# Aedelon/MASt3R-SLAM

Hardware: AMD Instinct MI355X
Metric: keyframe-pairs/sec (512x512 two-view infer+match+GN) (higher is better)
Workload: dtype fp16

## Files before the change

### include/m3slam_model.h

```cpp
#ifndef M3SLAM_MODEL_H
#define M3SLAM_MODEL_H

#include <stdint.h>

#ifdef __cplusplus
extern "C" {
#endif

enum { M3_DT_BF16 = 0, M3_DT_F16 = 1, M3_DT_F16_PVBF16 = 2 };

enum {
    M3_EPI_BF16 = 0,
    M3_EPI_BF16_GELU = 1,
    M3_EPI_F32 = 2,
    M3_EPI_F32_ACCUM = 3,
    M3_EPI_BF16_RELU = 4,
    M3_EPI_BF16_ADD = 5,
    M3_EPI_BF16_ROPE = 6,
    M3_EPI_INPUT_RELU = 0x100
};

typedef struct m3_gemm_desc {
    const void *A, *W, *W1;
    const float *bias, *bias1;
    void *C;
    const void *R;
    const int32_t *rope_pos;
    void *c16;
    float *stats_out;
    const float *ln_stats, *ln_colsum, *ln_colsum1;
    const void *r_lo;
    void *c_lo;
    int64_t a_gstride, c_gstride, ln_gstride, stats_gstride;
    int32_t M, N, K, ldc, epilogue, dtype, groups;
    int32_t tokens_per_image, rope_cols, q_cols, ln_slots;
    float rope_base, q_scale, ln_eps;
    int32_t stats_slots;
    int32_t rope_max_pos;
} m3_gemm_desc;
int m3_gemm_ex(const m3_gemm_desc *desc, void *stream);
int m3_gemm_pick_tile(int M, int N, int groups);
int m3_gemm_set_tile(int tile);
int m3_ln_slot_count(int M, int N, int groups);

int m3_conv3x3_grouped2_dt(const void *X, const void *W0, const void *W1, const float *bias0, const float *bias1,
                           void *Y, const void *R, const void *zero16, int B, int H, int Wd, int Cin, int Cout,
                           int stride, int epilogue, void *splitk_ws, int64_t splitk_ws_bytes, int dtype,
                           void *stream);

int64_t m3_conv3x3_splitk_bytes(int B, int H, int Wd, int Cin, int Cout, int stride);

int m3_conv3x3_relu_head4_dt(const void *X, const void *W, const float *bias, const void *W4, const float *b4,
                             float *pts, float *conf, const void *zero16, int B, int H, int Wd, int Cin,
                             int dtype, void *stream);

int m3_dpt_tail_grouped2_dt(const void *X, const void *Wc0, const void *Wc1, const float *bias0, const float *bias1,
                            const void *W40, const void *W41, const float *b40, const float *b41, float *pts,
                            float *conf, const void *zero16, int B, int H, int Wd, int upsample, int dtype,
                            void *stream);

int m3_conv3x3_up_direct_grouped2_dt(const void *X, const void *W0, const void *W1, const float *bias0,
                                     const float *bias1, void *Y, const void *zero16, int B, int H, int Wd, int Cin,
                                     int upsample, int dtype, void *stream);

int m3_conv3x3_direct_grouped2_dt(const void *X, const void *W0, const void *W1, const float *bias0, const float *bias1,
                                  void *Y, const void *R, const void *zero16, int B, int H, int Wd, int Cin, int Cout,
                                  int epilogue, int dtype, void *stream);

int m3_attention_dt(const void *Q, const void *K, const void *V, void *O, int q_row_stride,
                    int kv_row_stride, int o_row_stride, int64_t q_batch_stride,
                    int64_t kv_batch_stride, int64_t o_batch_stride, int nbatch, int heads,
                    int Tq, int Tk, int kv_batch_shift, float scale, int dtype, void *stream);

int m3_attention_prescaled_dt(const void *Q, const void *K, const void *V, void *O, int q_row_stride,
                              int kv_row_stride, int o_row_stride, int64_t q_batch_stride,
                              int64_t kv_batch_stride, int64_t o_batch_stride, int nbatch, int heads,
                              int Tq, int Tk, int kv_batch_shift, int dtype, void *stream);

int m3_rope2d_dt(void *X, const int32_t *pos_yx, const float *cos_sin, int row_stride, int tokens,
                 int heads, int tokens_per_image, int dtype, void *stream);

int m3_layernorm_dt(const float *x, const float *gamma, const float *beta, void *y, int M, int C,
                    float eps, int dtype, void *stream);

int m3_layernorm_grouped2_dt(const float *x, const float *gamma0, const float *beta0, const float *gamma1,
                             const float *beta1, void *y, int M, int C, int in_row_shift, float eps,
                             int dtype, void *stream);
int m3_layernorm_hl_dt(const void *hi, const void *lo, const float *gamma0, const float *beta0, const float *gamma1,
                       const float *beta1, void *y, int rows, int C, int split, float eps, int dtype, void *stream);
int m3_layernorm_dual2_dt(const float *x, const float *ga0, const float *ba0, const float *ga1, const float *ba1,
                          const float *gb0, const float *bb0, const float *gb1, const float *bb1, void *y_own,
                          void *y_cross, int M, int C, float eps, int dtype, void *stream);

int m3_patchify16_dt(const uint8_t *img, void *A, int B, int H, int W, int dtype, void *stream);

int m3_cast_f32_dt(const float *x, void *y, int64_t n, int dtype, void *stream);
int m3_cast16(const void *x, void *y, int64_t n, int from_dtype, int to_dtype, void *stream);
int m3_relu_bf16(const void *x, void *y, int64_t n, void *stream);
int m3_add_dt(const void *a, const void *b, void *y, int64_t n, int dtype, void *stream);
int m3_concat2_bf16(const void *a, const void *b, void *out, int64_t M, int Ca, int Cb, void *stream);
typedef struct m3_pack_seg { const void *src; int64_t dst_off; int64_t nbytes; int32_t mode; int32_t reserved; } m3_pack_seg;
int m3_pack_fields(void *dst, const m3_pack_seg *segs, int nseg, void *stream);
int m3_unshuffle_bf16(const void *in, void *out, int B, int h, int w, int s, int C, int Cpad, void *stream);
int m3_upsample2x_dt(const void *in, void *out, int B, int H, int W, int C, int dtype, void *stream);
int m3_add_upsample2x_dt(const void *low, const void *y, void *out, int B, int H, int W, int OH, int OW, int C,
                         int dtype, void *stream);
int m3_pts_post(const float *in, float *pts, float *conf, int64_t P, void *stream);
int m3_desc_post_dt(const void *in, float *desc, float *dconf, int B, int H, int W, int dtype, void *stream);
int m3_desc_post_f16(const void *in, void *desc_f16, float *dconf, int B, int H, int W, int dtype, void *stream);

#ifdef __cplusplus
}
#endif
#endif
```

### mast3r-slam_amd/csrc/gemm.hip

```cpp
#include <atomic>
#include "gemm_common.h"
#include <cmath>
#include <stdlib.h>

using namespace m3gemm;

namespace {

constexpr int BM = 128, BN = 128;
constexpr int kThreads = 256;

#ifndef M3_GEMM64_STAGES
#define M3_GEMM64_STAGES 2
#endif
constexpr int k_gemm_stages(int T) { return T == 64 ? M3_GEMM64_STAGES : 2; }

template <int MODE , int EPI, int T, int DT, bool SLICED = false>
__global__ void __launch_bounds__(kThreads)
k_gemm(const GemmArgs gin) {
    constexpr int BM = T, BN = T;
    constexpr int NT = T / 32;
    constexpr int kStageBytes = (BM + BN) * BK * 2;
    constexpr int STAGES = k_gemm_stages(T);
    static_assert(4 * (NT == 4 ? 9216 : 4608) + BM * 8 + kRopeTableRows * 128 <= STAGES * kStageBytes, "row table + RoPE table behind the scratch");
    GemmArgs g = select_group<EPI>(gin, blockIdx.y);
    extern __shared__ __attribute__((aligned(16))) unsigned char lds[];
    const int tid = threadIdx.x, lane = tid & 63, wave = tid >> 6;
    const int wr = wave >> 1, wc = wave & 1;
    int kt0 = 0, nk = g.K / BK;
    if (EPI == EPI_F32 && g.splits > 1) {
        const int all = nk, s = blockIdx.z;
        kt0 = (int)((long long)all * s / g.splits);
        nk = (int)((long long)all * (s + 1) / g.splits) - kt0;
        g.C = reinterpret_cast<float *>(g.C) + (size_t)s * g.M * g.ldc;
    }

    const int tiles_n = (g.N + BN - 1) / BN, tiles_m = (g.M + BM - 1) / BM;
    const int nwg = tiles_m * tiles_n;
    const int bid = xcd_remap(blockIdx.x, nwg);
    const int tm = bid / tiles_n, tn = bid % tiles_n;
    const int m0 = tm * BM, n0 = tn * BN;

    const int srow = tid >> 3, sch = (tid & 7) ^ ((srow >> 1) & 7);
    const bf16_t *a_src[NT];
    const bf16_t *w_src[NT];
    int a_oy[NT], a_ox[NT];
    const bf16_t *a_img[NT];
#pragma unroll
    for (int i = 0; i < NT; ++i) {
        int m = m0 + i * 32 + srow;
        m = m < g.M ? m : g.M - 1;
        int n = n0 + i * 32 + srow;
        n = n < g.N ? n : g.N - 1;
        w_src[i] = g.W + (size_t)n * g.K + sch * 8;
        if (MODE == 0) {
            a_src[i] = g.A + (size_t)m * g.K + sch * 8;
        } else {
            const int pix = g.OH * g.OW;
            const int b = m / pix, rem = m - b * pix;
            a_oy[i] = (rem / g.OW) * g.stride - 1;
            a_ox[i] = (rem % g.OW) * g.stride - 1;
            a_img[i] = g.A + (size_t)b * g.H * g.Wd * g.Cin + sch * 8;
        }
    }
    auto stage = [&](int kt, int buf) {
        kt += kt0;
        unsigned char *base = lds + buf * kStageBytes;
        int ky = 0, kx = 0, c0 = 0;
        if (MODE == 1) {
            const int q = kt / 9, tap = kt - q * 9;
            c0 = q * BK;
            ky = tap / 3; kx = tap - ky * 3;
        }
#pragma unroll
        for (int i = 0; i < NT; ++i) {
            const void *src;
            if (MODE == 0) {
                src = a_src[i] + (size_t)kt * BK;
            } else {
                const int iy = a_oy[i] + ky, ix = a_ox[i] + kx;
                const bool in = (iy >= 0) && (iy < g.H) && (ix >= 0) && (ix < g.Wd);
                src = in ? (const void *)(a_img[i] + ((size_t)iy * g.Wd + ix) * g.Cin + c0) : (const void *)g.zero16;
            }
            glds16(src, base + i * 4096 + wave * 1024);
        }
        const size_t koff = MODE == 1 ? conv_k_offset(kt, g.Cin) : (size_t)kt * BK;
#pragma unroll
        for (int i = 0; i < NT; ++i)
            glds16(w_src[i] + koff, base + BM * BK * 2 + i * 4096 + wave * 1024);
    };

    f32x4 acc[NT][NT];
#pragma unroll
    for (int i = 0; i < NT; ++i)
#pragma unroll
        for (int j = 0; j < NT; ++j) acc[i][j] = f32x4{0.f, 0.f, 0.f, 0.f};

    const int frow = lane & 15, fch = lane >> 4;

    constexpr bool CAN_SLICE = SLICED;
    static_assert(!SLICED || (MODE == 1 && T == 128), "sliced accumulation: convolutions on 128 x 128 tiles");
    f32x4 tot[CAN_SLICE ? NT : 1][CAN_SLICE ? NT : 1];
    const int slices = CAN_SLICE ? g.slices : 1;
    int slice = 0, slice_end = slices > 1 ? (int)((long long)nk * 1 / slices) : nk;

    float4 ln_mr = make_float4(0.f, 0.f, 0.f, 0.f);
    if (MODE == 0 && g.ln_stats) {
        const LnLoads L = ln_row_issue<BM>(g, m0, tid);
#pragma unroll
        for (int t0 = 0; t0 < STAGES - 1; ++t0)
            if (t0 < nk) stage(t0, t0);
        ln_mr = ln_row_finish<BM>(g, L, m0, tid);
    } else {
#pragma unroll
        for (int t0 = 0; t0 < STAGES - 1; ++t0)
            if (t0 < nk) stage(t0, t0);
    }
    for (int kt = 0; kt < nk; ++kt) {
        const int buf = kt & (STAGES - 1);
        if (kt + STAGES - 1 < nk) stage(kt + STAGES - 1, (kt + STAGES - 1) & (STAGES - 1));
        const int ahead = nk - 1 - kt < STAGES - 1 ? nk - 1 - kt : STAGES - 1;
        if constexpr (STAGES == 2) {
            if (ahead) {
                if constexpr (NT == 4) asm volatile("s_waitcnt vmcnt(8)" ::: "memory");
                else asm volatile("s_waitcnt vmcnt(4)" ::: "memory");
            } else asm volatile("s_waitcnt vmcnt(0)" ::: "memory");
        } else {
            static_assert(STAGES == 2 || (STAGES == 4 && NT == 2), "vmcnt immediates below are for 4 loads per tile");
            if (ahead == 3) asm volatile("s_waitcnt vmcnt(12)" ::: "memory");
            else if (ahead == 2) asm volatile("s_waitcnt vmcnt(8)" ::: "memory");
            else if (ahead == 1) asm volatile("s_waitcnt vmcnt(4)" ::: "memory");
            else asm volatile("s_waitcnt vmcnt(0)" ::: "memory");
        }
        lds_barrier();
        const unsigned char *As = lds + buf * kStageBytes;
        const unsigned char *Ws = As + BM * BK * 2;
#pragma unroll
        for (int ks = 0; ks < 2; ++ks) {
            bf16x8 af[NT], wf[NT];
#pragma unroll
            for (int i = 0; i < NT; ++i) {
                const int ra = wr * (T / 2) + i * 16 + frow;
                const int ca = (ks * 4 + fch) ^ ((ra >> 1) & 7);
                af[i] = *reinterpret_cast<const bf16x8 *>(As + ra * 128 + ca * 16);
                const int rw = wc * (T / 2) + i * 16 + frow;
                const int cw = (ks * 4 + fch) ^ ((rw >> 1) & 7);
                wf[i] = *reinterpret_cast<const bf16x8 *>(Ws + rw * 128 + cw * 16);
            }
            if (MODE == 1 && g.relu_a) {
#pragma unroll
                for (int i = 0; i < NT; ++i) af[i] = relu_frag(af[i]);
            }
#pragma unroll
            for (int i = 0; i < NT; ++i)
#pragma unroll
                for (int j = 0; j < NT; ++j)
                    acc[i][j] = mfma16<DT>(wf[j], af[i], acc[i][j]);
        }
        lds_barrier();
        if constexpr (CAN_SLICE) {
            if (slices > 1 && kt + 1 == slice_end) {
#pragma unroll
                for (int i = 0; i < NT; ++i)
#pragma unroll
                    for (int j = 0; j < NT; ++j) {
                        tot[i][j] = slice == 0 ? acc[i][j] : tot[i][j] + acc[i][j];
                        acc[i][j] = f32x4{0.f, 0.f, 0.f, 0.f};
                    }
                ++slice;
                slice_end = (int)((long long)nk * (slice + 1) / slices);
            }
        }
    }
    if constexpr (CAN_SLICE) {
        if (slices > 1) {
#pragma unroll
            for (int i = 0; i < NT; ++i)
#pragma unroll
                for (int j = 0; j < NT; ++j) acc[i][j] = tot[i][j];
        }
    }

    if constexpr (EPI == EPI_RELU_HEAD4) {
        static_assert(T == 128, "head fusion needs the 128-wide tile");
        const int r = lane & 15, gq = lane >> 4;
        float part[NT][4];
#pragma unroll
        for (int i = 0; i < NT; ++i)
#pragma unroll
            for (int o = 0; o < 4; ++o) part[i][o] = 0.f;
#pragma unroll
        for (int j = 0; j < NT; ++j) {
            const int n = wc * 64 + j * 16 + gq * 4;
            const float4 b = g.bias ? *reinterpret_cast<const float4 *>(g.bias + n) : make_float4(0.f, 0.f, 0.f, 0.f);
            float w4[4][4];
#pragma unroll
            for (int o = 0; o < 4; ++o) {
                const uint2 q = *reinterpret_cast<const uint2 *>(g.W2 + (size_t)o * g.N + n);
                w4[o][0] = lo16<DT>(q.x); w4[o][1] = hi16<DT>(q.x); w4[o][2] = lo16<DT>(q.y); w4[o][3] = hi16<DT>(q.y);
            }
#pragma unroll
            for (int i = 0; i < NT; ++i) {
                const f32x4 a = acc[i][j];
                const float h[4] = {fmaxf(a[0] + b.x, 0.f), fmaxf(a[1] + b.y, 0.f), fmaxf(a[2] + b.z, 0.f), fmaxf(a[3] + b.w, 0.f)};
#pragma unroll
                for (int o = 0; o < 4; ++o)
                    part[i][o] += (h[0] * w4[o][0] + h[1] * w4[o][1]) + (h[2] * w4[o][2] + h[3] * w4[o][3]);
            }
        }
#pragma unroll
        for (int i = 0; i < NT; ++i)
#pragma unroll
            for (int o = 0; o < 4; ++o) {
                float v = part[i][o];
                v += __shfl_xor(v, 16, 64);
                v += __shfl_xor(v, 32, 64);
                part[i][o] = v;
            }
        float *red = reinterpret_cast<float *>(lds);
        if (wc == 1 && gq == 0) {
#pragma unroll
            for (int i = 0; i < NT; ++i)
                *reinterpret_cast<float4 *>(red + (wr * 64 + i * 16 + r) * 4) =
                    make_float4(part[i][0], part[i][1], part[i][2], part[i][3]);
        }
        __syncthreads();
        if (wc == 0 && gq == 0) {
            float *pts = reinterpret_cast<float *>(g.C);
#pragma unroll
            for (int i = 0; i < NT; ++i) {
                const int m = m0 + wr * 64 + i * 16 + r;
                if (m >= g.M) continue;
                const float4 q = *reinterpret_cast<const float4 *>(red + (wr * 64 + i * 16 + r) * 4);
                const float x = part[i][0] + q.x + g.bias2[0], y = part[i][1] + q.y + g.bias2[1];
                const float z = part[i][2] + q.z + g.bias2[2], c = part[i][3] + q.w + g.bias2[3];
                const float d = sqrtf(x * x + y * y + z * z);
                const float sc = expm1f(d) / fmaxf(d, 1e-8f);
                pts[3 * (size_t)m + 0] = x * sc; pts[3 * (size_t)m + 1] = y * sc; pts[3 * (size_t)m + 2] = z * sc;
                g.C2[m] = 1.0f + expf(c);
            }
        }
    } else {
        float2 *lnt = nullptr;
        if (MODE == 0 && g.ln_stats) {
            lnt = reinterpret_cast<float2 *>(lds + 4 * (NT == 4 ? 9216 : 4608));
            ln_table_store<BM>(lnt, ln_mr, tid);
            __syncthreads();
        }
        const float *ropet = nullptr;
        if constexpr (EPI == EPI_BF16_ROPE && MODE == 0) {
            if (g.rope_pos && g.rope_pmax > 0) {
                float *tab = reinterpret_cast<float *>(lds + 4 * (NT == 4 ? 9216 : 4608) + BM * 8);
                rope_table_build(g, tab, tid, kThreads);
                __syncthreads();
                ropet = tab;
            }
        }
        epilogue_rows<EPI, NT, NT, DT, (EPI == EPI_BF16_ROPE && T == 128) ? 2 : 4>(g, acc, lds + wave * (NT == 4 ? 9216 : 4608), m0 + wr * (T / 2),
                                                                                  n0 + wc * (T / 2), lane, lnt, wr * (T / 2), ropet);
        if constexpr (MODE == 0 && (EPI == EPI_F32 || EPI == EPI_F32_ACCUM)) {
            if (g.stats_out) {
                __syncthreads();
                stats_tile_finalize<BM, NT, NT, 2>(g, lds, NT == 4 ? 9216 : 4608, stats_stage_offset<NT>(), m0, n0, tid);
            }
        }
    }
}

template <int MODE, int T, int DT>
int launch_dt(const GemmArgs &a, int epi, hipStream_t st) {
    constexpr int kLdsBytes = k_gemm_stages(T) * (2 * T) * BK * 2;
    const int tiles = m3_cdiv(a.M, T) * m3_cdiv(a.N, T);
    dim3 grid(tiles, a.groups > 1 ? a.groups : 1, a.splits > 1 ? a.splits : 1), blk(kThreads);
#define M3_L(E) case E: hipLaunchKernelGGL((k_gemm<MODE, E, T, DT>), grid, blk, kLdsBytes, st, a); break
    if (a.slices > 1) {
        if constexpr (MODE == 1 && T == 128) {
            switch (epi) {
                case EPI_BF16: hipLaunchKernelGGL((k_gemm<1, EPI_BF16, 128, DT, true>), grid, blk, kLdsBytes, st, a); break;
                case EPI_BF16_RELU: hipLaunchKernelGGL((k_gemm<1, EPI_BF16_RELU, 128, DT, true>), grid, blk, kLdsBytes, st, a); break;
                case EPI_BF16_ADD: hipLaunchKernelGGL((k_gemm<1, EPI_BF16_ADD, 128, DT, true>), grid, blk, kLdsBytes, st, a); break;
                default: return M3_ERR_INVALID_ARG;
            }
        } else return M3_ERR_INVALID_ARG;
    } else
    if (epi == EPI_RELU_HEAD4) {
        if constexpr (MODE == 1 && T == 128) hipLaunchKernelGGL((k_gemm<1, EPI_RELU_HEAD4, 128, DT>), grid, blk, kLdsBytes, st, a);
        else return M3_ERR_INVALID_ARG;
    } else
    switch (epi) {
        M3_L(EPI_BF16); M3_L(EPI_BF16_GELU); M3_L(EPI_F32); M3_L(EPI_F32_ACCUM); M3_L(EPI_BF16_RELU); M3_L(EPI_BF16_ADD); M3_L(EPI_BF16_ROPE);
        default: return M3_ERR_INVALID_ARG;
    }
#undef M3_L
    M3_CHECK_LAUNCH("m3_gemm");
    return M3_OK;
}

template <int MODE, int T = 128>
int launch(const GemmArgs &a, int epi, hipStream_t st) {
    return a.dt == DT_F16 ? launch_dt<MODE, T, DT_F16>(a, epi, st) : launch_dt<MODE, T, DT_BF16>(a, epi, st);
}

static const double kCost64 = [] { const char *e = getenv("M3_GEMM_COST64"); return e ? atof(e) : 3.2; }();
static std::atomic<int> g_forced_tile{[] { const char *e = getenv("M3_GEMM_TILE"); return e ? atoi(e) : 0; }()};
int pick_tile(int M, int N, int groups = 1, bool dense = true) {
    const int forced = g_forced_tile.load(std::memory_order_relaxed);
    const bool can192 = dense && N % 192 == 0;
    if (forced == 128 || forced == 256) return forced;
    if (forced == 192) return can192 ? 192 : 256;
    const long t256 = (long)m3_cdiv(M, 256) * m3_cdiv(N, 256) * groups, t128 = (long)m3_cdiv(M, 128) * m3_cdiv(N, 128) * groups;
    const double c256 = (double)((t256 + 255) / 256) * 4.0 / 1.4, c128 = (double)((t128 + 511) / 512) * 2.0;
    double c192 = 1e30;
    if (can192) {
        const long t192 = (long)m3_cdiv(M, 256) * (N / 192) * groups;
        c192 = (double)((t192 + 255) / 256) * 3.0 / 1.4 * 1.02;
    }
    double c64 = 1e30;
    if (dense) {
        const long t64 = (long)m3_cdiv(M, 64) * m3_cdiv(N, 64) * groups;
        c64 = (double)((t64 + 1023) / 1024) * 2.0 * 0.25 * kCost64;
    }
    if (forced == 64) return dense ? 64 : 128;
    if (c64 < c128 && c64 < c256 && c64 < c192) return 64;
    if (c192 < c256 && c192 < c128) return 192;
    return c256 < c128 ? 256 : 128;
}
bool use_256(int M, int N, int groups = 1) { return pick_tile(M, N, groups, false) == 256; }

int pick_splits(int pix_per_image, int N, int K) {
    const long tiles = (long)m3_cdiv(pix_per_image, BM) * m3_cdiv(N, BN);
    const int nk = K / BK;
    if (nk < 8) return 1;
    long s = 64 / tiles;
    if (s > nk / 4) s = nk / 4;
    if (s > 16) s = 16;
    return s < 2 ? 1 : (int)s;
}

template <int EPI, int DT>
__global__ void __launch_bounds__(256)
k_splitk_finish(const GemmArgs gin, const float *__restrict__ part, int S) {
    const GemmArgs g = select_group<EPI>(gin, blockIdx.y);
    part += (size_t)blockIdx.y * S * gin.M * gin.N;
    const int nq = g.N / 4;
    const long q = (long)blockIdx.x * 256 + threadIdx.x;
    const int m = (int)(q / nq), n = (int)(q - (long)m * nq) * 4;
    if (m >= g.M) return;
    const size_t plane = (size_t)g.M * g.N;
    const float *p = part + (size_t)m * g.N + n;
    float4 a = *reinterpret_cast<const float4 *>(p);
    for (int s = 1; s < S; ++s) {
        const float4 b = *reinterpret_cast<const float4 *>(p + s * plane);
        a.x += b.x; a.y += b.y; a.z += b.z; a.w += b.w;
    }
    store_tile<EPI, DT>(g, f32x4{a.x, a.y, a.z, a.w}, m, n);
}

template <int MODE>
int run_split(const GemmArgs &a, int S, int epi, void *ws, hipStream_t st) {
    if (MODE == 1 && (epi == EPI_BF16 || epi == EPI_BF16_RELU || epi == EPI_BF16_ADD)) {
        const long tiles = (long)m3_cdiv(a.M, BM) * m3_cdiv(a.N, BN) * (a.groups > 1 ? a.groups : 1);
        static const bool sliced_ok = [] { const char *e = getenv("M3_CONV_SLICED"); return !(e && atoi(e) == 0); }();
        if (sliced_ok && tiles >= m3_device_cu_count()) {
            GemmArgs q = a;
            q.slices = S; q.splits = 1;
            return launch<MODE>(q, epi, st);
        }
    }
    GemmArgs p = a;
    p.C = ws; p.ldc = a.N; p.bias = nullptr; p.bias2 = nullptr; p.R = nullptr; p.splits = S;
    p.c_gstride = (long long)S * a.M * a.N;
    const int rc = launch<MODE>(p, EPI_F32, st);
    if (rc != M3_OK) return rc;
    const dim3 grid((unsigned)m3_cdiv((long)a.M * (a.N / 4), 256L), a.groups > 1 ? a.groups : 1);
#define M3_F(E) case E:                                                                                        \
        if (a.dt == DT_F16) hipLaunchKernelGGL((k_splitk_finish<E, DT_F16>), grid, dim3(256), 0, st, a, (const float *)ws, S); \
        else hipLaunchKernelGGL((k_splitk_finish<E, DT_BF16>), grid, dim3(256), 0, st, a, (const float *)ws, S);      \
        break
    switch (epi) {
        M3_F(EPI_BF16); M3_F(EPI_BF16_GELU); M3_F(EPI_F32); M3_F(EPI_F32_ACCUM); M3_F(EPI_BF16_RELU); M3_F(EPI_BF16_ADD);
        default: return M3_ERR_INVALID_ARG;
    }
#undef M3_F
    M3_CHECK_LAUNCH("m3_gemm/splitk_finish");
    return M3_OK;
}

}

int m3_launch_gemm256_dense(const GemmArgs &a, int epi, int bn, hipStream_t st);
int m3_launch_gemm256_conv(const GemmArgs &a, int epi, hipStream_t st);

static int launch_dense(const GemmArgs &a, int epi, hipStream_t st) {
    const int tile = pick_tile(a.M, a.N, a.groups > 1 ? 2 : 1);
    if (tile >= 192) return m3_launch_gemm256_dense(a, epi, tile, st);
    if (tile == 64) return launch<0, 64>(a, epi, st);
    return launch<0>(a, epi, st);
}

extern "C" {

int m3_gemm_set_tile(int tile) { return g_forced_tile.exchange(tile, std::memory_order_relaxed); }

int m3_gemm_pick_tile(int M, int N, int groups) {
    if (M <= 0 || N <= 0) return 0;
    return pick_tile(M, N, groups > 1 ? groups : 1);
}

static bool dt_ok(int dtype) { return dtype == DT_BF16 || dtype == DT_F16; }

static int ln_top_width(int C) {
    if (C % 192 == 0 && C / 192 <= 4) return 192;
    if (C % 256 == 0 && C / 256 <= 4) return 256;
    return 0;
}
static int ln_store_width(int M, int N, int groups) {
    const int tile = pick_tile(M, N, groups), top = ln_top_width(N);
    if (top == 0) return 0;
    if (tile == top) return top;
    if (top == 256 && tile == 128) return 128;
    return 64;
}
int m3_ln_slot_count(int M, int N, int groups) {
    if (M <= 0 || N <= 0) return 0;
    const int w = ln_store_width(M, N, groups > 1 ? 2 : 1);
    return w ? N / w : 0;
}

int m3_gemm_ex(const m3_gemm_desc *d, void *stream) {
    M3_REQUIRE(d && d->A && d->W && (d->C || d->c_lo) && d->M > 0 && d->N > 0 && d->K > 0);
    const int epi = d->epilogue, groups = d->groups > 1 ? 2 : 1;
    const bool rope = epi == EPI_BF16_ROPE;
    M3_REQUIRE(dt_ok(d->dtype) || (rope && d->dtype == 2));
    M3_REQUIRE(d->K % BK == 0 && d->N % 4 == 0 && d->ldc >= d->N && d->ldc % 4 == 0);
    M3_REQUIRE(!((epi == EPI_F32_ACCUM || epi == EPI_BF16_ADD) && !d->R));
    M3_REQUIRE(epi >= EPI_BF16 && epi <= EPI_BF16_ROPE);
    if (d->c_lo)
        M3_REQUIRE((epi == EPI_F32 || epi == EPI_F32_ACCUM) && d->dtype == DT_F16 && d->c16 && !d->C && d->N % 8 == 0 && d->ldc % 8 == 0 &&
                   d->M % 2 == 0 && (reinterpret_cast<size_t>(d->c_lo) & 15) == 0 && (reinterpret_cast<size_t>(d->c16) & 15) == 0 &&
                   (epi == EPI_F32 || (d->r_lo && (reinterpret_cast<size_t>(d->R) & 15) == 0 && (reinterpret_cast<size_t>(d->r_lo) & 15) == 0)));
    if (groups == 2) M3_REQUIRE(d->W1 && (d->bias == nullptr) == (d->bias1 == nullptr));
    if (rope)
        M3_REQUIRE(d->rope_pos && d->tokens_per_image > 0 && d->rope_base > 1.0f && d->N % 64 == 0 && d->rope_cols % 64 == 0 &&
                   d->rope_cols <= d->N && d->q_cols >= 0 && d->q_cols <= d->rope_cols && d->q_cols % 64 == 0);
    const bool f32out = epi == EPI_F32 || epi == EPI_F32_ACCUM;
    if (d->c16 || d->stats_out) {
        M3_REQUIRE(f32out && (d->N % 64 == 0 || !d->stats_out) && d->M % 2 == 0 && d->ldc % 8 == 0 && (reinterpret_cast<size_t>(d->C) & 15) == 0 &&
                   (!d->R || (reinterpret_cast<size_t>(d->R) & 15) == 0) &&
                   (!d->c16 || (reinterpret_cast<size_t>(d->c16) & 15) == 0) &&
                   (!d->stats_out || (reinterpret_cast<size_t>(d->stats_out) & 15) == 0));
        if (groups == 2) M3_REQUIRE(d->c_gstride % 8 == 0 && d->stats_gstride % 4 == 0);
        if (d->stats_out) M3_REQUIRE(d->stats_slots > 0 && d->stats_slots == m3_ln_slot_count(d->M, d->N, groups));
    }
    if (d->ln_stats) {
        const int top = ln_top_width(d->K);
        M3_REQUIRE(top != 0 && (d->ln_slots == d->K / 64 || (top == 256 && d->ln_slots == d->K / 128) || d->ln_slots == d->K / top));
        M3_REQUIRE(!f32out && epi != EPI_BF16_ADD && d->ln_colsum &&
                   d->ln_eps > 0.0f && d->M % 2 == 0 && (reinterpret_cast<size_t>(d->ln_stats) & 15) == 0 &&
                   (reinterpret_cast<size_t>(d->ln_colsum) & 15) == 0 && (reinterpret_cast<size_t>(d->C) & 15) == 0 &&
                   d->ldc % 8 == 0 && d->N % 8 == 0);
        if (groups == 2) M3_REQUIRE(d->ln_colsum1 && (reinterpret_cast<size_t>(d->ln_colsum1) & 15) == 0 && d->ln_gstride % 4 == 0);
    }
    GemmArgs a{};
    a.A = (const bf16_t *)d->A; a.W = (const bf16_t *)d->W; a.W2 = (const bf16_t *)d->W1; a.bias = d->bias; a.bias2 = d->bias1;
    a.C = d->C; a.R = d->R; a.M = d->M; a.N = d->N; a.K = d->K; a.ldc = d->ldc;
    a.dt = d->dtype == 2 ? DT_F16 : d->dtype; a.v_bf16 = d->dtype == 2;
    a.a_gstride = d->a_gstride; a.c_gstride = d->c_gstride; a.groups = groups == 2 ? 2 : 0;
    if (rope) {
        a.rope_pos = d->rope_pos; a.rope_log2_base = log2f(d->rope_base); a.tokens_per_image = d->tokens_per_image;
        a.rope_cols = d->rope_cols; a.q_cols = d->q_cols; a.q_scale = d->q_scale;
        a.rope_pmax = (d->rope_max_pos > 0 && d->rope_max_pos <= kRopeTableRows) ? d->rope_max_pos : 0;
    }
    a.C16 = d->c16; a.stats_out = d->stats_out; a.stats_gstride = d->stats_gstride;
    a.R_lo = d->r_lo; a.C_lo = d->c_lo;
    a.ln_stats = d->ln_stats; a.ln_colsum = d->ln_colsum; a.ln_colsum2 = d->ln_colsum1; a.ln_slots = d->ln_slots;
    a.ln_eps = d->ln_eps; a.ln_gstride = d->ln_gstride;
    if (d->ln_stats) {
        const int top = ln_top_width(d->K);
        a.ln_tops = d->K / top;
        a.ln_gsz = d->ln_slots / a.ln_tops;
    }
    a.stats_w = d->stats_out ? ln_store_width(d->M, d->N, groups) : 0;
    return launch_dense(a, epi, (hipStream_t)stream);
}

int64_t m3_conv3x3_splitk_bytes(int B, int H, int Wd, int Cin, int Cout, int stride) {
    if (B <= 0 || H <= 0 || Wd <= 0 || Cin <= 0 || Cout <= 0 || (stride != 1 && stride != 2)) return 0;
    const int OH = (H + 2 - 3) / stride + 1, OW = (Wd + 2 - 3) / stride + 1;
    const int S = pick_splits(OH * OW, Cout, 9 * Cin);
    return S > 1 ? (int64_t)S * B * OH * OW * Cout * 4 : 0;
}

int m3_conv3x3_grouped2_dt(const void *X, const void *W0, const void *W1, const float *bias0, const float *bias1,
                           void *Y, const void *R, const void *zero16, int B, int H, int Wd, int Cin, int Cout,
                           int stride, int epilogue, void *splitk_ws, int64_t splitk_ws_bytes, int dtype, void *stream) {
    const int relu_in = (epilogue & 0x100) ? 1 : 0;
    epilogue &= 0xff;
    M3_REQUIRE(X && W0 && Y && zero16 && B > 0 && H > 0 && Wd > 0 && Cin > 0 && Cout > 0 && dt_ok(dtype));
    M3_REQUIRE(Cin % BK == 0 && Cout % 4 == 0 && (stride == 1 || stride == 2) && epilogue != EPI_BF16_ROPE);
    M3_REQUIRE(!((epilogue == EPI_F32_ACCUM || epilogue == EPI_BF16_ADD) && !R));
    M3_REQUIRE(!W1 || (bias0 == nullptr) == (bias1 == nullptr));
    GemmArgs a{};
    a.relu_a = relu_in;
    a.A = (const bf16_t *)X; a.W = (const bf16_t *)W0; a.bias = bias0; a.C = Y; a.R = R;
    a.zero16 = (const bf16_t *)zero16;
    a.H = H; a.Wd = Wd; a.Cin = Cin; a.stride = stride;
    a.OH = (H + 2 - 3) / stride + 1; a.OW = (Wd + 2 - 3) / stride + 1;
    a.M = B * a.OH * a.OW; a.N = Cout; a.K = 9 * Cin; a.ldc = Cout; a.dt = dtype;
    if (W1) {
        a.W2 = (const bf16_t *)W1; a.bias2 = bias1;
        a.groups = 2; a.a_gstride = (long long)B * H * Wd * Cin; a.c_gstride = (long long)a.M * Cout;
    }
    const int S = pick_splits(a.OH * a.OW, Cout, a.K);
    if (S > 1) {
        M3_REQUIRE(splitk_ws && (reinterpret_cast<size_t>(splitk_ws) & 15) == 0 &&
                   splitk_ws_bytes >= (W1 ? 2 : 1) * (int64_t)S * a.M * a.N * 4);
        return run_split<1>(a, S, epilogue, splitk_ws, (hipStream_t)stream);
    }
    if (use_256(a.M, a.N, W1 ? 2 : 1)) return m3_launch_gemm256_conv(a, epilogue, (hipStream_t)stream);
    return launch<1>(a, epilogue, (hipStream_t)stream);
}

int m3_conv3x3_relu_head4_dt(const void *X, const void *W, const float *bias, const void *W4, const float *b4,
                             float *pts, float *conf, const void *zero16, int B, int H, int Wd, int Cin, int dtype,
                             void *stream) {
    M3_REQUIRE(X && W && W4 && b4 && pts && conf && zero16 && B > 0 && H > 0 && Wd > 0 && Cin > 0 && Cin % BK == 0);
    M3_REQUIRE(dt_ok(dtype));
    M3_REQUIRE((int64_t)B * H * Wd < (1ll << 31));
    GemmArgs a{};
    a.A = (const bf16_t *)X; a.W = (const bf16_t *)W; a.bias = bias; a.C = pts; a.C2 = conf;
    a.W2 = (const bf16_t *)W4; a.bias2 = b4;
    a.zero16 = (const bf16_t *)zero16;
    a.H = H; a.Wd = Wd; a.Cin = Cin; a.stride = 1; a.OH = H; a.OW = Wd;
    a.M = B * H * Wd; a.N = 128; a.K = 9 * Cin; a.ldc = 3; a.dt = dtype;
    return launch<1>(a, EPI_RELU_HEAD4, (hipStream_t)stream);
}

}
```

### mast3r-slam_amd/csrc/gemm256.hip

```cpp
#include "gemm_common.h"

using namespace m3gemm;

namespace {

constexpr int BM = 256;
constexpr int kThreads = 512;

template <int MODE , int EPI, int BN, int DT>
__global__ void __launch_bounds__(kThreads, 2)
k_gemm256(const GemmArgs gin) {
    constexpr int WN = BN == 256 ? 4 : 2, WM = 8 / WN;
    constexpr int NI = BM / WM / 16, NJ = BN / WN / 16;
    constexpr int WISS = BN / 64;
    constexpr int kStageBytes = (BM + BN) * BK * 2;
    static_assert(8 * (64 * (32 * NJ + 16)) + kRopeTableRows * 128 <= 2 * kStageBytes, "RoPE table behind the epilogue scratch");
    const GemmArgs g = select_group<EPI>(gin, blockIdx.y);
    extern __shared__ __attribute__((aligned(16))) unsigned char lds[];
    const int tid = threadIdx.x, lane = tid & 63, wave = tid >> 6;
    const int group = wave >> 2;
    const int wr = wave / WN, wc = wave % WN;

    const int tiles_n = (g.N + BN - 1) / BN, tiles_m = (g.M + BM - 1) / BM;
    const int bid = xcd_remap(blockIdx.x, tiles_m * tiles_n);
    constexpr int GM = 8;
    const int band = bid / (GM * tiles_n), first_m = band * GM;
    const int gsz = tiles_m - first_m < GM ? tiles_m - first_m : GM;
    const int in_band = bid - band * GM * tiles_n;
    const int tm = first_m + in_band % gsz, tn = in_band / gsz;
    const int m0 = tm * BM, n0 = tn * BN;

    const int srow = tid >> 3, sch = (tid & 7) ^ ((srow >> 1) & 7);
    const bf16_t *a_src[4];
    const bf16_t *w_src[WISS];
    int a_oy[4], a_ox[4];
    const bf16_t *a_img[4];
#pragma unroll
    for (int i = 0; i < WISS; ++i) {
        int n = n0 + i * 64 + srow;
        n = n < g.N ? n : g.N - 1;
        w_src[i] = g.W + (size_t)n * g.K + sch * 8;
    }
#pragma unroll
    for (int i = 0; i < 4; ++i) {
        int m = m0 + i * 64 + srow;
        m = m < g.M ? m : g.M - 1;
        if (MODE == 0) {
            a_src[i] = g.A + (size_t)m * g.K + sch * 8;
        } else {
            const int pix = g.OH * g.OW;
            const int b = m / pix, rem = m - b * pix;
            a_oy[i] = (rem / g.OW) * g.stride - 1;
            a_ox[i] = (rem % g.OW) * g.stride - 1;
            a_img[i] = g.A + (size_t)b * g.H * g.Wd * g.Cin + sch * 8;
        }
    }
    const int nk = g.K / BK;

    auto stage_a = [&](int kt, int buf) {
        unsigned char *base = lds + buf * kStageBytes;
        int ky = 0, kx = 0, c0 = 0;
        if (MODE == 1) {
            const int q = kt / 9, tap = kt - q * 9;
            c0 = q * BK;
            ky = tap / 3; kx = tap - ky * 3;
        }
#pragma unroll
        for (int i = 0; i < 4; ++i) {
            const void *src;
            if (MODE == 0) {
                src = a_src[i] + (size_t)kt * BK;
            } else {
                const int iy = a_oy[i] + ky, ix = a_ox[i] + kx;
                const bool in = (iy >= 0) && (iy < g.H) && (ix >= 0) && (ix < g.Wd);
                src = in ? (const void *)(a_img[i] + ((size_t)iy * g.Wd + ix) * g.Cin + c0) : (const void *)g.zero16;
            }
            glds16(src, base + i * 8192 + wave * 1024);
        }
    };
    auto stage_w = [&](int kt, int buf) {
        unsigned char *base = lds + buf * kStageBytes;
        const size_t koff = MODE == 1 ? conv_k_offset(kt, g.Cin) : (size_t)kt * BK;
#pragma unroll
        for (int i = 0; i < WISS; ++i)
            glds16(w_src[i] + koff, base + BM * BK * 2 + i * 8192 + wave * 1024);
    };
    auto stage = [&](int kt, int buf) { stage_a(kt, buf); stage_w(kt, buf); };

    f32x4 acc[NI][NJ];
#pragma unroll
    for (int i = 0; i < NI; ++i)
#pragma unroll
        for (int j = 0; j < NJ; ++j) acc[i][j] = f32x4{0.f, 0.f, 0.f, 0.f};

    const int frow = lane & 15, fch = lane >> 4;
    int a_off[NI], w_off[NJ];
#pragma unroll
    for (int i = 0; i < NI; ++i) {
        const int r = wr * (16 * NI) + i * 16 + frow;
        a_off[i] = r * 128 + ((fch ^ ((r >> 1) & 7)) << 4);
    }
#pragma unroll
    for (int j = 0; j < NJ; ++j) {
        const int r = wc * (16 * NJ) + j * 16 + frow;
        w_off[j] = BM * BK * 2 + r * 128 + ((fch ^ ((r >> 1) & 7)) << 4);
    }

    bf16x8 af[NI], wf[NJ];
    auto read_frags = [&](int buf, int ks) {
        const unsigned char *base = lds + buf * kStageBytes;
#pragma unroll
        for (int j = 0; j < NJ; ++j) wf[j] = *reinterpret_cast<const bf16x8 *>(base + (w_off[j] ^ (ks << 6)));
#pragma unroll
        for (int i = 0; i < NI; ++i) af[i] = *reinterpret_cast<const bf16x8 *>(base + (a_off[i] ^ (ks << 6)));
        if (MODE == 1 && g.relu_a) {
#pragma unroll
            for (int i = 0; i < NI; ++i) af[i] = relu_frag(af[i]);
        }
    };
    auto mfma_all = [&]() {
        __builtin_amdgcn_s_setprio(1);
#pragma unroll
        for (int i = 0; i < NI; ++i)
#pragma unroll
            for (int j = 0; j < NJ; ++j)
                acc[i][j] = mfma16<DT>(wf[j], af[i], acc[i][j]);
        __builtin_amdgcn_s_setprio(0);
    };
    auto phase_end = [&]() {
        __builtin_amdgcn_sched_barrier(0);
        __builtin_amdgcn_s_barrier();
        __builtin_amdgcn_sched_barrier(0);
    };
    auto phase_end_wait = [&]() {
        __builtin_amdgcn_sched_barrier(0);
        asm volatile("s_waitcnt vmcnt(0)" ::: "memory");
        __builtin_amdgcn_s_barrier();
        __builtin_amdgcn_sched_barrier(0);
    };

    if (MODE == 0 && g.ln_stats) {
        float2 *lnt = reinterpret_cast<float2 *>(lds + 2 * kStageBytes);
        const LnLoads L = ln_row_issue<BM>(g, m0, tid);
        stage(0, 0);
        ln_table_store<BM>(lnt, ln_row_finish<BM>(g, L, m0, tid), tid);
    } else {
        stage(0, 0);
    }
    float2 *lnt = (MODE == 0 && g.ln_stats) ? reinterpret_cast<float2 *>(lds + 2 * kStageBytes) : nullptr;
    phase_end_wait();

    if (group == 0) {
        for (int kt = 0; kt < nk; ++kt) {
            const int buf = kt & 1;
            read_frags(buf, 0);
            if (kt + 1 < nk) stage_a(kt + 1, buf ^ 1);
            asm volatile("s_waitcnt lgkmcnt(0)" ::: "memory");
            phase_end();
            mfma_all();
            phase_end();
            read_frags(buf, 1);
            if (kt + 1 < nk) stage_w(kt + 1, buf ^ 1);
            asm volatile("s_waitcnt lgkmcnt(0)" ::: "memory");
            phase_end();
            mfma_all();
            phase_end_wait();
        }
        phase_end();
    } else {
        for (int kt = 0; kt < nk; ++kt) {
            const int buf = kt & 1;
            if (kt > 0) mfma_all();
            phase_end();
            read_frags(buf, 0);
            if (kt + 1 < nk) stage_a(kt + 1, buf ^ 1);
            asm volatile("s_waitcnt lgkmcnt(0)" ::: "memory");
            phase_end();
            if (kt + 1 < nk) stage_w(kt + 1, buf ^ 1);
            mfma_all();
            phase_end();
            read_frags(buf, 1);
            asm volatile("s_waitcnt lgkmcnt(0)" ::: "memory");
            phase_end_wait();
        }
        mfma_all();
        phase_end();
    }

    const float *ropet = nullptr;
    if constexpr (EPI == EPI_BF16_ROPE && MODE == 0) {
        if (g.rope_pos && g.rope_pmax > 0) {
            float *tab = reinterpret_cast<float *>(lds + 8 * (64 * (32 * NJ + 16)));
            rope_table_build(g, tab, tid, kThreads);
            __syncthreads();
            ropet = tab;
        }
    }
    epilogue_rows<EPI, NI, NJ, DT>(g, acc, lds + wave * (64 * (32 * NJ + 16)), m0 + wr * (16 * NI), n0 + wc * (16 * NJ), lane, lnt,
                                   wr * (16 * NI), ropet);
    if constexpr (MODE == 0 && (EPI == EPI_F32 || EPI == EPI_F32_ACCUM)) {
        if (g.stats_out) {
            __syncthreads();
            stats_tile_finalize<BM, NI, NJ, WN>(g, lds, 64 * (32 * NJ + 16), stats_stage_offset<NJ>(), m0, n0, tid);
        }
    }
}

template <int MODE, int BN, int DT>
int launch256(const GemmArgs &a, int epi, hipStream_t st) {
    constexpr int kLdsBytes = 2 * (BM + BN) * BK * 2 + BM * 8;
    const int tiles = m3_cdiv(a.M, BM) * m3_cdiv(a.N, BN);
    dim3 grid(tiles, a.groups > 1 ? a.groups : 1), blk(kThreads);
#define M3_L(E)                                                                                              \
    case E: {                                                                                                \
        static M3AttrOnce once;                                                                              \
        int dev__;                                                                                           \
        if (m3_attr_need(once, &dev__)) {                                                                    \
            M3_CHECK_HIP(hipFuncSetAttribute(reinterpret_cast<const void *>(&k_gemm256<MODE, E, BN, DT>),        \
                                             hipFuncAttributeMaxDynamicSharedMemorySize, kLdsBytes),         \
                         "m3_gemm256/attr");                                                                 \
            m3_attr_done(once, dev__);                                                                       \
        }                                                                                                    \
        hipLaunchKernelGGL((k_gemm256<MODE, E, BN, DT>), grid, blk, kLdsBytes, st, a);                           \
    } break
    switch (epi) {
        M3_L(EPI_BF16); M3_L(EPI_BF16_GELU); M3_L(EPI_F32); M3_L(EPI_F32_ACCUM); M3_L(EPI_BF16_RELU); M3_L(EPI_BF16_ADD); M3_L(EPI_BF16_ROPE);
        default: return M3_ERR_INVALID_ARG;
    }
#undef M3_L
    M3_CHECK_LAUNCH("m3_gemm256");
    return M3_OK;
}

}

int m3_launch_gemm256_dense(const GemmArgs &a, int epi, int bn, hipStream_t st) {
    if (a.dt == DT_F16) return bn == 192 ? launch256<0, 192, DT_F16>(a, epi, st) : launch256<0, 256, DT_F16>(a, epi, st);
    return bn == 192 ? launch256<0, 192, DT_BF16>(a, epi, st) : launch256<0, 256, DT_BF16>(a, epi, st);
}
int m3_launch_gemm256_conv(const GemmArgs &a, int epi, hipStream_t st) {
    return a.dt == DT_F16 ? launch256<1, 256, DT_F16>(a, epi, st) : launch256<1, 256, DT_BF16>(a, epi, st);
}
```

Measured before the change: 283.3.

## Build RoPE table in GEMM prologue and split dense GEMMs by column for wave balance

The RoPE table build moves from after the K loop to the prologue, into dedicated extra LDS past the stage buffers. This overlaps the build with the first tile loads and drops the barrier before the epilogue, at the cost of more LDS per block and possibly lower occupancy. Dense GEMMs with a small tail wave are also split by columns: a leading part runs on 256/192 tiles and the remainder on 128 tiles, chosen by a heuristic cost model, to cut tail-wave waste. A new API can force the split point.

```diff
diff --git a/include/m3slam_model.h b/include/m3slam_model.h
--- a/include/m3slam_model.h
+++ b/include/m3slam_model.h
@@ -41,6 +41,8 @@
 int m3_gemm_ex(const m3_gemm_desc *desc, void *stream);
 int m3_gemm_pick_tile(int M, int N, int groups);
 int m3_gemm_set_tile(int tile);
+int m3_gemm_pick_nsplit(int M, int N, int groups);
+int m3_gemm_set_nsplit(int lead_cols);
 int m3_ln_slot_count(int M, int N, int groups);
 
 int m3_conv3x3_grouped2_dt(const void *X, const void *W0, const void *W1, const float *bias0, const float *bias1,
diff --git a/mast3r-slam_amd/csrc/gemm.hip b/mast3r-slam_amd/csrc/gemm.hip
--- a/mast3r-slam_amd/csrc/gemm.hip
+++ b/mast3r-slam_amd/csrc/gemm.hip
@@ -22,7 +22,8 @@
     constexpr int NT = T / 32;
     constexpr int kStageBytes = (BM + BN) * BK * 2;
     constexpr int STAGES = k_gemm_stages(T);
-    static_assert(4 * (NT == 4 ? 9216 : 4608) + BM * 8 + kRopeTableRows * 128 <= STAGES * kStageBytes, "row table + RoPE table behind the scratch");
+    constexpr bool ROPE_PRO = EPI == EPI_BF16_ROPE && MODE == 0 && T == 128;
+    static_assert(4 * (NT == 4 ? 9216 : 4608) + BM * 8 + (ROPE_PRO ? 0 : kRopeTableRows * 128) <= STAGES * kStageBytes, "row table (+ RoPE table) behind the scratch");
     GemmArgs g = select_group<EPI>(gin, blockIdx.y);
     extern __shared__ __attribute__((aligned(16))) unsigned char lds[];
     const int tid = threadIdx.x, lane = tid & 63, wave = tid >> 6;
@@ -115,6 +116,14 @@
 #pragma unroll
         for (int t0 = 0; t0 < STAGES - 1; ++t0)
             if (t0 < nk) stage(t0, t0);
+    }
+    const float *ropet = nullptr;
+    if constexpr (ROPE_PRO) {
+        if (g.rope_pos && g.rope_pmax > 0) {
+            float *tab = reinterpret_cast<float *>(lds + STAGES * kStageBytes);
+            rope_table_build(g, tab, tid, kThreads);
+            ropet = tab;
+        }
     }
     for (int kt = 0; kt < nk; ++kt) {
         const int buf = kt & (STAGES - 1);
@@ -247,8 +256,7 @@
             ln_table_store<BM>(lnt, ln_mr, tid);
             __syncthreads();
         }
-        const float *ropet = nullptr;
-        if constexpr (EPI == EPI_BF16_ROPE && MODE == 0) {
+        if constexpr (EPI == EPI_BF16_ROPE && MODE == 0 && !ROPE_PRO) {
             if (g.rope_pos && g.rope_pmax > 0) {
                 float *tab = reinterpret_cast<float *>(lds + 4 * (NT == 4 ? 9216 : 4608) + BM * 8);
                 rope_table_build(g, tab, tid, kThreads);
@@ -273,6 +281,21 @@
     const int tiles = m3_cdiv(a.M, T) * m3_cdiv(a.N, T);
     dim3 grid(tiles, a.groups > 1 ? a.groups : 1, a.splits > 1 ? a.splits : 1), blk(kThreads);
 #define M3_L(E) case E: hipLaunchKernelGGL((k_gemm<MODE, E, T, DT>), grid, blk, kLdsBytes, st, a); break
+    if constexpr (MODE == 0 && T == 128) {
+        if (epi == EPI_BF16_ROPE && a.slices <= 1) {
+            constexpr int kRopeLds = kLdsBytes + kRopeTableRows * 128;
+            static M3AttrOnce once;
+            int dev;
+            if (m3_attr_need(once, &dev)) {
+                M3_CHECK_HIP(hipFuncSetAttribute(reinterpret_cast<const void *>(&k_gemm<0, EPI_BF16_ROPE, 128, DT>),
+                                                 hipFuncAttributeMaxDynamicSharedMemorySize, kRopeLds), "m3_gemm/attr");
+                m3_attr_done(once, dev);
+            }
+            hipLaunchKernelGGL((k_gemm<0, EPI_BF16_ROPE, 128, DT>), grid, blk, kRopeLds, st, a);
+            M3_CHECK_LAUNCH("m3_gemm");
+            return M3_OK;
+        }
+    }
     if (a.slices > 1) {
         if constexpr (MODE == 1 && T == 128) {
             switch (epi) {
@@ -326,6 +349,22 @@
     return c256 < c128 ? 256 : 128;
 }
 bool use_256(int M, int N, int groups = 1) { return pick_tile(M, N, groups, false) == 256; }
+
+static std::atomic<int> g_forced_nsplit{0};
+int pick_nsplit(int M, int N, int groups, int bn) {
+    if (bn != 256 && bn != 192) return 0;
+    const long tm = (long)m3_cdiv(M, 256) * groups, cols = m3_cdiv(N, bn), tiles = tm * cols;
+    const long full = tiles / 256, rem = tiles % 256;
+    if (full == 0 || rem == 0 || rem * 2 >= 256) return 0;
+    const long lead_cols = full * 256 / tm;
+    if (lead_cols < 1 || lead_cols >= cols) return 0;
+    const int lead = (int)lead_cols * bn;
+    const double per_round = (bn == 192 ? 3.0 * 1.02 : 4.0) / 1.4;
+    const long t128 = (long)m3_cdiv(M, 128) * m3_cdiv(N - lead, 128) * groups;
+    const double one = (double)(full + 1) * per_round;
+    const double two = (double)((tm * lead_cols + 255) / 256) * per_round + (double)((t128 + 511) / 512) * 2.0;
+    return two < one ? lead : 0;
+}
 
 int pick_splits(int pix_per_image, int N, int K) {
     const long tiles = (long)m3_cdiv(pix_per_image, BM) * m3_cdiv(N, BN);
@@ -391,8 +430,35 @@
 int m3_launch_gemm256_dense(const GemmArgs &a, int epi, int bn, hipStream_t st);
 int m3_launch_gemm256_conv(const GemmArgs &a, int epi, hipStream_t st);
 
+static GemmArgs column_range(const GemmArgs &a, int epi, int n0, int n) {
+    GemmArgs s = a;
+    const size_t esz = (epi == EPI_F32 || epi == EPI_F32_ACCUM) ? 4 : 2;
+    s.N = n;
+    s.W = a.W + (size_t)n0 * a.K;
+    if (a.W2) s.W2 = a.W2 + (size_t)n0 * a.K;
+    if (a.bias) s.bias = a.bias + n0;
+    if (a.bias2) s.bias2 = a.bias2 + n0;
+    s.C = reinterpret_cast<unsigned char *>(a.C) + (size_t)n0 * esz;
+    if (a.R) s.R = reinterpret_cast<const unsigned char *>(a.R) + (size_t)n0 * esz;
+    if (a.ln_colsum) s.ln_colsum = a.ln_colsum + n0;
+    if (a.ln_colsum2) s.ln_colsum2 = a.ln_colsum2 + n0;
+    return s;
+}
+
 static int launch_dense(const GemmArgs &a, int epi, hipStream_t st) {
-    const int tile = pick_tile(a.M, a.N, a.groups > 1 ? 2 : 1);
+    const int groups = a.groups > 1 ? 2 : 1;
+    if (epi != EPI_BF16_ROPE && !a.stats_out && !a.C16 && !a.C_lo && g_forced_tile.load(std::memory_order_relaxed) == 0) {
+        const int forced = g_forced_nsplit.load(std::memory_order_relaxed);
+        const int t = pick_tile(a.M, a.N, groups);
+        const int bn = forced > 0 ? 256 : t;
+        const int lead = forced > 0 ? forced : pick_nsplit(a.M, a.N, groups, t);
+        if (lead > 0 && lead < a.N && lead % bn == 0) {
+            const int rc = m3_launch_gemm256_dense(column_range(a, epi, 0, lead), epi, bn, st);
+            if (rc != M3_OK) return rc;
+            return launch<0>(column_range(a, epi, lead, a.N - lead), epi, st);
+        }
+    }
+    const int tile = pick_tile(a.M, a.N, groups);
     if (tile >= 192) return m3_launch_gemm256_dense(a, epi, tile, st);
     if (tile == 64) return launch<0, 64>(a, epi, st);
     return launch<0>(a, epi, st);
@@ -405,6 +471,14 @@
 int m3_gemm_pick_tile(int M, int N, int groups) {
     if (M <= 0 || N <= 0) return 0;
     return pick_tile(M, N, groups > 1 ? groups : 1);
+}
+
+int m3_gemm_set_nsplit(int lead_cols) { return g_forced_nsplit.exchange(lead_cols > 0 ? lead_cols : 0, std::memory_order_relaxed); }
+
+int m3_gemm_pick_nsplit(int M, int N, int groups) {
+    if (M <= 0 || N <= 0) return 0;
+    const int g = groups > 1 ? 2 : 1;
+    return pick_nsplit(M, N, g, pick_tile(M, N, g));
 }
 
 static bool dt_ok(int dtype) { return dtype == DT_BF16 || dtype == DT_F16; }
diff --git a/mast3r-slam_amd/csrc/gemm256.hip b/mast3r-slam_amd/csrc/gemm256.hip
--- a/mast3r-slam_amd/csrc/gemm256.hip
+++ b/mast3r-slam_amd/csrc/gemm256.hip
@@ -14,7 +14,8 @@
     constexpr int NI = BM / WM / 16, NJ = BN / WN / 16;
     constexpr int WISS = BN / 64;
     constexpr int kStageBytes = (BM + BN) * BK * 2;
-    static_assert(8 * (64 * (32 * NJ + 16)) + kRopeTableRows * 128 <= 2 * kStageBytes, "RoPE table behind the epilogue scratch");
+    static_assert(8 * (64 * (32 * NJ + 16)) <= 2 * kStageBytes, "the waves' epilogue scratch lives in the dead stages");
+    constexpr bool ROPE = EPI == EPI_BF16_ROPE && MODE == 0;
     const GemmArgs g = select_group<EPI>(gin, blockIdx.y);
     extern __shared__ __attribute__((aligned(16))) unsigned char lds[];
     const int tid = threadIdx.x, lane = tid & 63, wave = tid >> 6;
@@ -148,6 +149,15 @@
         stage(0, 0);
     }
     float2 *lnt = (MODE == 0 && g.ln_stats) ? reinterpret_cast<float2 *>(lds + 2 * kStageBytes) : nullptr;
+    const float *ropet = nullptr;
+    if constexpr (ROPE) {
+        if (g.rope_pos && g.rope_pmax > 0) {
+            float *tab = reinterpret_cast<float *>(lds + 2 * kStageBytes + BM * 8);
+            rope_table_build(g, tab, tid, kThreads);
+            ropet = tab;
+            asm volatile("s_waitcnt lgkmcnt(0)" ::: "memory");
+        }
+    }
     phase_end_wait();
 
     if (group == 0) {
@@ -187,15 +197,6 @@
         phase_end();
     }
 
-    const float *ropet = nullptr;
-    if constexpr (EPI == EPI_BF16_ROPE && MODE == 0) {
-        if (g.rope_pos && g.rope_pmax > 0) {
-            float *tab = reinterpret_cast<float *>(lds + 8 * (64 * (32 * NJ + 16)));
-            rope_table_build(g, tab, tid, kThreads);
-            __syncthreads();
-            ropet = tab;
-        }
-    }
     epilogue_rows<EPI, NI, NJ, DT>(g, acc, lds + wave * (64 * (32 * NJ + 16)), m0 + wr * (16 * NI), n0 + wc * (16 * NJ), lane, lnt,
                                    wr * (16 * NI), ropet);
     if constexpr (MODE == 0 && (EPI == EPI_F32 || EPI == EPI_F32_ACCUM)) {
@@ -208,11 +209,12 @@
 
 template <int MODE, int BN, int DT>
 int launch256(const GemmArgs &a, int epi, hipStream_t st) {
-    constexpr int kLdsBytes = 2 * (BM + BN) * BK * 2 + BM * 8;
+    constexpr int kLdsBase = 2 * (BM + BN) * BK * 2 + BM * 8;
     const int tiles = m3_cdiv(a.M, BM) * m3_cdiv(a.N, BN);
     dim3 grid(tiles, a.groups > 1 ? a.groups : 1), blk(kThreads);
 #define M3_L(E)                                                                                              \
     case E: {                                                                                                \
+        constexpr int kLdsBytes = kLdsBase + (MODE == 0 && E == EPI_BF16_ROPE ? kRopeTableRows * 128 : 0);   \
         static M3AttrOnce once;                                                                              \
         int dev__;                                                                                           \
         if (m3_attr_need(once, &dev__)) {                                                                    \
```

After: 285.0, median of 6. About the same (+0.6%).
